# mika314/melonix

Measured on AMD Instinct MI355X. Metric: STFT+pitch+resynth frames/sec (48 kHz, 4096 FFT, 256 hop); % HBM roofline, higher is better.
Workload: dtype f32

## Files before the change

### melonix_amd/csrc/stft_core.h

```cpp
#pragma once
#include <stdint.h>
#include <type_traits>

#if defined(__HIPCC__)
#include <hip/hip_runtime.h>
#define MX_HD __host__ __device__ __forceinline__
namespace mx {
using cpx = float2;
}
#else
#define MX_HD inline __attribute__((always_inline))
namespace mx {
struct alignas(8) cpx {
  float x, y;
};
}
#endif

namespace mx {

#include "stft_consts.inc"

MX_HD cpx mk(float x, float y) {
  cpx r;
// ... 203 lines not shown
    for (int e = 0; e < P::E; ++e) {
      const cpx xs = ld_pair<ALIGNED8>(x, 2 * (t + P::T * e));
      Y[e] = pk_mul(xs, e < P::E - kGeoTail ? geo_weight<P, false>(a0, e) : geo_weight<P, true>(a0, e));
    }
  } else {
#pragma unroll
    for (int e = 0; e < P::E; ++e) Y[e] = pk_mul(ld_pair<ALIGNED8>(x, 2 * (t + P::T * e)), geo_weight<P, true>(a0, e));
  }
}

template <class P>
MX_HD void apply_window_geo(int t, cpx (&Y)[P::E], const cpx (&xr)[P::E], const float *wb, int hop) {
  const cpx a0 = ld_pair<true>(wb, 2 * t);
  if (geo_clamped_slots<P>(hop) <= kGeoTail) {
#pragma unroll
    for (int e = 0; e < P::E; ++e)
      Y[e] = pk_mul(xr[e], e < P::E - kGeoTail ? geo_weight<P, false>(a0, e) : geo_weight<P, true>(a0, e));
  } else {
#pragma unroll
    for (int e = 0; e < P::E; ++e) Y[e] = pk_mul(xr[e], geo_weight<P, true>(a0, e));
  }
}

template <class P, bool ALIGNED8>
MX_HD void load_raw(int t, cpx (&xr)[P::E], const float *x) {
#pragma unroll
  for (int e = 0; e < P::E; ++e) {
    xr[e] = ld_pair<ALIGNED8>(x, 2 * (t + P::T * e));
  }
}
template <class P, int WSTEP, bool ALIGNED8>
MX_HD void apply_window(int t, cpx (&Y)[P::E], const cpx (&xr)[P::E], const float *w) {
#pragma unroll
  for (int e = 0; e < P::E; ++e) {
    const int p = 2 * (t + P::T * e);
    cpx ws;
    if constexpr (WSTEP == 1) {
      ws = ld_pair<ALIGNED8>(w, p);
    } else {
      const f2u wu = *reinterpret_cast<const f2u *>(w - p - 1);
      ws = mk(wu.y, wu.x);
    }
    Y[e] = pk_mul(xr[e], ws);
  }
}

template <class P>
MX_HD void pass1(const cpx (&Y)[P::E], cpx (&v)[P::E]) {
#pragma unroll
  for (int b = 0; b < P::NB1; ++b) {
    cpx in[P::R1], out[P::R1];
#pragma unroll
    for (int r = 0; r < P::R1; ++r) in[r] = Y[b + P::NB1 * r];
    Dft<P::R1>::run(in, out);
#pragma unroll
    for (int r = 0; r < P::R1; ++r) v[b * P::R1 + r] = out[r];
  }
}

template <class P, int HOP>
struct Slide {
  static constexpr int H = HOP / 2;
  static constexpr bool ok = (HOP > 0) && (HOP % 2 == 0) && (H % P::T == 0) && (2 * (H / P::T) <= P::E);
  static constexpr int D = ok ? H / P::T : 1;
};

template <class P, int HOP>
MX_HD void slide_edge(int t, const float *wtab, float inv_sc, cpx (&edge)[Slide<P, HOP>::D]) {
  using S = Slide<P, HOP>;
#pragma unroll
  for (int i = 0; i < S::D; ++i) {
    const int p = 2 * (t + P::T * (P::E - 2 * S::D + i));
    edge[i] = mk(wtab[p] * inv_sc, wtab[p + 1] * inv_sc);
  }
}

template <class P, int HOP>
MX_HD void slide_fetch(int t, const float *xe, cpx (&nx)[Slide<P, HOP>::D]) {
  using S = Slide<P, HOP>;
#pragma unroll
  for (int i = 0; i < S::D; ++i) nx[i] = *reinterpret_cast<const cpx *>(xe - HOP + 2 * (t + P::T * i));
}

template <class P, int HOP>
MX_HD void slide_step(cpx (&Y)[P::E], const cpx (&nx)[Slide<P, HOP>::D], const cpx (&edge)[Slide<P, HOP>::D],
                      float g, float sc) {
  using S = Slide<P, HOP>;
  const cpx gg = mk(g, g), ss = mk(sc, sc);
#pragma unroll
  for (int e = 0; e < P::E - 2 * S::D; ++e) Y[e] = pk_mul_xs(Y[e + S::D], gg);
#pragma unroll
  for (int i = 0; i < S::D; ++i) Y[P::E - 2 * S::D + i] = pk_mul(Y[P::E - S::D + i], edge[i]);
#pragma unroll
  for (int i = 0; i < S::D; ++i) Y[P::E - S::D + i] = pk_mul_xs(nx[i], ss);
}


template <class P>
struct Circ {
  static constexpr int W = 2 * P::T;
  static constexpr int CS = (P::T == 128) ? 4 : (P::T == 256) ? 3 : 2;
  static MX_HD bool ok(int hop) { return hop >= 1 && hop <= (CS - 1) * P::T && hop <= 2 * W; }
  static constexpr int slot(int k) { return (P::E - (CS - 1) + k) & (P::E - 1); }
};
template <class P>
struct CircGeo {
  int o;
  int s;
  int cr;
  int len;
};
template <class P>
MX_HD CircGeo<P> circ_geo(long long frame_end, int hop) {
  constexpr int W = Circ<P>::W;
  const long long start = frame_end - P::N;
  CircGeo<P> g;
  g.o = (int)(start & (long long)(W - 1));
  g.s = ((int)((start - hop) & (long long)(W - 1)) + hop) / W;
  g.len = 2 * hop;
  g.cr = (g.o - g.len) & (P::N - 1);
  return g;
}
template <class P>
MX_HD void circ_load_first(int t, cpx (&Y)[P::E], const float *xa, const float *w, int o) {
#pragma unroll
  for (int e = 0; e < P::E; ++e) {
    const int c2 = 2 * (t + P::T * e);
    const int q0 = (c2 - o) & (P::N - 1), q1 = (c2 + 1 - o) & (P::N - 1);
    Y[e] = mk(xa[q0] * w[q0], xa[q1] * w[q1]);
  }
}
template <class P>
MX_HD void circ_fetch(int t, const float *xs, const float *wt, const CircGeo<P> &g, float (&px)[2 * Circ<P>::CS],
                      float (&pw)[2 * Circ<P>::CS]) {
#pragma unroll
  for (int k = 0; k < Circ<P>::CS; ++k) {
    const int c2 = 2 * (t + P::T * Circ<P>::slot(k));
    int d0 = (c2 - g.cr) & (P::N - 1), d1 = (c2 + 1 - g.cr) & (P::N - 1);
    d0 = d0 < g.len ? d0 : g.len - 1;
    d1 = d1 < g.len ? d1 : g.len - 1;
    px[2 * k] = ld_one(xs, d0);
    px[2 * k + 1] = ld_one(xs, d1);
    pw[2 * k] = ld_one(wt, d0);
    pw[2 * k + 1] = ld_one(wt, d1);
  }
}
template <class P, int S>
MX_HD void circ_age(cpx (&Y)[P::E], cpx gg) {
  cpx head[S > 0 ? S : 1];
#pragma unroll
  for (int i = 0; i < S; ++i) head[i] = Y[i];
#pragma unroll
  for (int e = 0; e < P::E - S; ++e) Y[e] = pk_mul_xs(Y[e + S], gg);
#pragma unroll
  for (int i = 0; i < S; ++i) Y[P::E - S + i] = pk_mul_xs(head[i], gg);
}
template <class P>
MX_HD void circ_step(int t, cpx (&Y)[P::E], float decay, const CircGeo<P> &g, const float (&px)[2 * Circ<P>::CS],
                     const float (&pw)[2 * Circ<P>::CS]) {
  const cpx gg = mk(decay, decay);
  constexpr int SMAX = (Circ<P>::W - 1 + (Circ<P>::CS - 1) * P::T) / Circ<P>::W;
  static_assert(SMAX <= 2, "rotations by 0, 1 or 2 slots");
  if (g.s == 0) circ_age<P, 0>(Y, gg);
  else if (SMAX == 1 || g.s == 1) circ_age<P, 1>(Y, gg);
  else circ_age<P, 2>(Y, gg);
#pragma unroll
  for (int k = 0; k < Circ<P>::CS; ++k) {
    const int e = Circ<P>::slot(k);
    const int c2 = 2 * (t + P::T * e);
    const int d0 = (c2 - g.cr) & (P::N - 1), d1 = (c2 + 1 - g.cr) & (P::N - 1);
    const float n0 = px[2 * k] * pw[2 * k], n1 = px[2 * k + 1] * pw[2 * k + 1];
    Y[e] = mk(d0 < g.len ? n0 : Y[e].x, d1 < g.len ? n1 : Y[e].y);
  }
}


#if defined(__HIP_DEVICE_COMPILE__)
#define MX_LDS_ASM 1
typedef float mx_f2v __attribute__((ext_vector_type(2)));
template <int OFF>
__device__ __forceinline__ mx_f2v lds_rd64(uint32_t addr) {
  static_assert(OFF >= 0 && OFF < 163840, "LDS is 160 KiB");
  mx_f2v r;
  if constexpr (OFF < 65536) {
    asm volatile("ds_read_b64 %0, %1 offset:%2" : "=v"(r) : "v"(addr), "n"(OFF) : "memory");
  } else {
    const uint32_t hi = addr + (uint32_t)(OFF & ~65535);
    asm volatile("ds_read_b64 %0, %1 offset:%2" : "=v"(r) : "v"(hi), "n"(OFF & 65535) : "memory");
  }
  return r;
}
__device__ __forceinline__ uint32_t lds_addr(const void *p) {
  return (uint32_t)(uintptr_t)(const __attribute__((address_space(3))) void *)p;
}
template <int N>
__device__ __forceinline__ void lds_wait(mx_f2v (&q)[N]) {
  static_assert(N % 8 == 0, "tied in groups of 8");
  asm volatile("s_waitcnt lgkmcnt(0)" ::: "memory");
#pragma unroll
  for (int i = 0; i < N; i += 8)
    asm volatile("" : "+v"(q[i]), "+v"(q[i + 1]), "+v"(q[i + 2]), "+v"(q[i + 3]), "+v"(q[i + 4]),
                 "+v"(q[i + 5]), "+v"(q[i + 6]), "+v"(q[i + 7]));
}
#endif
template <int I, int N, class F>
MX_HD void static_for(F &&f) {
  if constexpr (I < N) {
    f(std::integral_constant<int, I>{});
    static_for<I + 1, N>(f);
  }
}

template <class P>
MX_HD void store_t1(int t, const cpx (&v)[P::E], cpx *lds) {
  if constexpr (t1_padded<P>()) {
    static_assert(P::R1 <= 32 && (P::T * P::R1) % 32 == 0, "T1 padding is one point per 32");
    cpx *const p = lds + (t * P::R1 + ((t * P::R1) >> 5));
#pragma unroll
    for (int b = 0; b < P::NB1; ++b) {
#pragma unroll
      for (int r = 0; r < P::R1; ++r) p[b * (P::T * P::R1 + P::T * P::R1 / 32) + r] = v[b * P::R1 + r];
    }
  } else {
    const unsigned B8 = (unsigned)((t * P::R1) ^ (t & 15)) << 3;
    char *const base = reinterpret_cast<char *>(lds);
#pragma unroll
    for (int r = 0; r < P::R1; ++r) {
      cpx *p = reinterpret_cast<cpx *>(base + (B8 ^ ((unsigned)r << 3)));
#pragma unroll
      for (int b = 0; b < P::NB1; ++b) p[b * P::T * P::R1] = v[b * P::R1 + r];
    }
  }
}

template <class P>
struct T1Read {
  static constexpr int S = P::M / P::R2;
  static constexpr int SP = t1_padded<P>() ? S + S / 32 : S;
  static constexpr int TP = t1_padded<P>() ? P::T + P::T / 32 : P::T;
  static constexpr int step = t1_padded<P>() ? 0 : ((S >> P::L1) & 15);
  static_assert(S % 32 == 0 && P::T % 32 == 0 && (step == 0 || step == 8), "T1 read is base(+alt base) + offset");
  static_assert(t1_padded<P>() || P::NB2 == 1, "the XOR layout's bases are written for one pass-2 butterfly per thread");
};

template <class P>
MX_HD void load_t1(int t, cpx (&v)[P::E], const cpx *lds) {
  using R = T1Read<P>;
  const int s1 = t1_index<P>(t);
#ifdef MX_LDS_ASM
  mx_f2v q[P::E];
  const uint32_t ae = lds_addr(lds + s1), ao = lds_addr(lds + (s1 ^ R::step));
  static_for<0, P::NB2>([&](auto bb) {
    constexpr int b = decltype(bb)::value;
    static_for<0, P::R2>([&](auto rr) {
      constexpr int r = decltype(rr)::value;
      q[b * P::R2 + r] = lds_rd64<(b * R::TP + r * R::SP) * 8>((r & 1) ? ao : ae);
    });
  });
  lds_wait(q);
#pragma unroll
  for (int i = 0; i < P::E; ++i) v[i] = mk(q[i].x, q[i].y);
#else
  const cpx *pe = lds + s1, *po = lds + (s1 ^ R::step);
#pragma unroll
  for (int b = 0; b < P::NB2; ++b) {
#pragma unroll
    for (int r = 0; r < P::R2; ++r) v[b * P::R2 + r] = ((r & 1) ? po : pe)[b * R::TP + r * R::SP];
  }
#endif
}

template <class P>
MX_HD void load_t1_tw2(int t, cpx (&v)[P::E], const cpx *lds, const cpx *ltw2, cpx (&w)[P::R2 - 1]) {
  static_assert(P::NB2 == 1 && P::E == P::R2 && P::E % 8 == 0, "one pass-2 butterfly per thread");
  using R = T1Read<P>;
  const int s1 = t1_index<P>(t);
#ifdef MX_LDS_ASM
  const uint32_t ae = lds_addr(lds + s1), ao = lds_addr(lds + (s1 ^ R::step));
  const uint32_t aw = lds_addr(ltw2 + (t & (P::R1 - 1)));
  mx_f2v q[2 * P::E];
  static_for<0, P::R2>([&](auto rr) {
    constexpr int r = decltype(rr)::value;
    q[r] = lds_rd64<r * R::SP * 8>((r & 1) ? ao : ae);
  });
  static_for<1, P::R2>([&](auto rr) {
    constexpr int r = decltype(rr)::value;
    q[P::E + r] = lds_rd64<(r - 1) * P::R1 * 8>(aw);
  });
  q[P::E] = mx_f2v{0.0f, 0.0f};
  lds_wait(q);
#pragma unroll
  for (int i = 0; i < P::E; ++i) v[i] = mk(q[i].x, q[i].y);
#pragma unroll
  for (int r = 1; r < P::R2; ++r) w[r - 1] = mk(q[P::E + r].x, q[P::E + r].y);
#else
  const cpx *pe = lds + s1, *po = lds + (s1 ^ R::step), *pw = ltw2 + (t & (P::R1 - 1));
#pragma unroll
  for (int r = 0; r < P::R2; ++r) v[r] = ((r & 1) ? po : pe)[r * R::SP];
#pragma unroll
  for (int r = 1; r < P::R2; ++r) w[r - 1] = pw[(r - 1) * P::R1];
#endif
}

template <class P>
MX_HD void pass2(int t, cpx (&v)[P::E], const cpx *tw2) {
#pragma unroll
  for (int b = 0; b < P::NB2; ++b) {
    const int j = t + P::T * b;
    const int k = j & (P::R1 - 1);
    cpx in[P::R2], w[P::R2], out[P::R2];
    w[0] = mk(1.0f, 0.0f);
#pragma unroll
    for (int r = 0; r < P::R2; ++r) in[r] = v[b * P::R2 + r];
#pragma unroll
    for (int r = 1; r < P::R2; ++r) {
      w[r] = tw2[(r - 1) * P::R1 + k];
    }
    DftTw<P::R2, 1, 0, false>::run(in, w, out);
#pragma unroll
    for (int r = 0; r < P::R2; ++r) v[b * P::R2 + r] = out[r];
  }
}

template <class P>
MX_HD void pass2_reg(cpx (&v)[P::E], const cpx (&w)[P::R2 - 1]) {
  static_assert(P::NB2 == 1, "one pass-2 butterfly per thread");
  cpx in[P::R2], ww[P::R2], out[P::R2];
  ww[0] = mk(1.0f, 0.0f);
#pragma unroll
  for (int r = 0; r < P::R2; ++r) in[r] = v[r];
#pragma unroll
  for (int r = 1; r < P::R2; ++r) ww[r] = w[r - 1];
  DftTw<P::R2, 1, 0, false>::run(in, ww, out);
#pragma unroll
  for (int r = 0; r < P::R2; ++r) v[r] = out[r];
}

template <class P>
MX_HD void store_t2(int t, const cpx (&v)[P::E], cpx *lds) {
#pragma unroll
  for (int b = 0; b < P::NB2; ++b) {
    const int j = t + P::T * b;
    const int k = j & (P::R1 - 1);
    const int base = (j - k) * P::R2 + k;
    cpx *p = lds + base;
#pragma unroll
    for (int r = 0; r < P::R2; ++r) p[r * P::R1] = v[b * P::R2 + r];
  }
}

template <class P>
MX_HD int k0p(int t) { return t; }
template <class P>
MX_HD int k0q(int t) { return t ? P::NS3 - t : P::NS3 / 2; }

template <class P>
MX_HD void load_t2(int t, cpx (&v)[P::E], const cpx *lds) {
  const int p = k0p<P>(t), q = k0q<P>(t);
#ifdef MX_LDS_ASM
  {
    const uint32_t pa = lds_addr(lds + p), qa = lds_addr(lds + q);
    mx_f2v w[P::E];
    static_for<0, P::R3>([&](auto rr) {
      constexpr int r = decltype(rr)::value;
      w[r] = lds_rd64<P::NS3 * r * 8>(pa);
      w[P::R3 + r] = lds_rd64<P::NS3 * r * 8>(qa);
    });
    lds_wait(w);
#pragma unroll
    for (int i = 0; i < P::E; ++i) v[i] = mk(w[i].x, w[i].y);
  }
#else
  const cpx *pp = lds + p, *qq = lds + q;
#pragma unroll
  for (int r = 0; r < P::R3; ++r) {
    v[r] = pp[P::NS3 * r];
    v[P::R3 + r] = qq[P::NS3 * r];
  }
#endif
}

template <class P>
MX_HD constexpr int q_index(int r) { return P::R3 + ((r + 1) & (P::R3 - 1)); }

template <class P>
MX_HD void fetch_tw3(int t, const cpx *tw3, cpx (&w)[P::R3 - 1]) {
  const int col = t ? t : P::NS3 / 2;
#pragma unroll
  for (int r = 1; r < P::R3; ++r) w[r - 1] = tw3[(r - 1) * P::NS3 + col];
}
template <class P>
MX_HD void fetch_tw3_bases(int t, const cpx *tw3, cpx (&wb)[6]) {
  static_assert(P::R3 == 16, "two-level pass-3 twiddles are written for radix 16");
  const int col = t ? t : P::NS3 / 2;
  constexpr int rr[6] = {1, 2, 3, 4, 8, 12};
#pragma unroll
  for (int i = 0; i < 6; ++i) wb[i] = tw3[(rr[i] - 1) * P::NS3 + col];
}
template <class P, bool MAY0>
MX_HD void pass3_reg(int t, cpx (&v)[P::E], const cpx (&w)[P::R3 - 1]);
template <class P, bool MAY0 = true>
MX_HD void pass3_bases(int t, cpx (&v)[P::E], const cpx (&wb)[6]) {
  cpx w[P::R3 - 1];
#pragma unroll
  for (int r = 1; r < P::R3; ++r) {
    const int hi = r >> 2, lo = r & 3;
    if (hi == 0) w[r - 1] = wb[lo - 1];
    else if (lo == 0) w[r - 1] = wb[2 + hi];
    else w[r - 1] = pk_cmul2(wb[2 + hi], wb[lo - 1]);
  }
  pass3_reg<P, MAY0>(t, v, w);
}
template <class P, int KH>
MX_HD void pass3_wp0(int t, const cpx (&w)[P::R3 - 1], cpx (&wph)[KH > 0 ? KH : 1]) {
  static_assert(KH >= 0 && KH <= P::R3 - 1, "at most every twiddle");
  wph[0] = mk(1.0f, 0.0f);
#pragma unroll
  for (int r = 1; r <= KH; ++r) wph[r - 1] = csel(t == 0, mk(1.0f, 0.0f), w[r - 1]);
}
template <class P, bool MAY0 = true, int KH = 0>
MX_HD void pass3_reg(int t, cpx (&v)[P::E], const cpx (&w)[P::R3 - 1], const cpx (&wph)[KH > 0 ? KH : 1]) {
  constexpr int R = P::R3;
  const bool t0 = MAY0 && (t == 0);
  cpx inp[R], inq[R], wp[R], wq[R], out[R];
  wp[0] = wq[0] = mk(1.0f, 0.0f);
#pragma unroll
  for (int r = 0; r < R; ++r) {
    inp[r] = v[r];
    inq[r] = v[R + r];
  }
#pragma unroll
  for (int r = 1; r < R; ++r) {
    wp[r] = (MAY0 && r <= KH) ? wph[r <= KH ? r - 1 : 0] : csel(t0, mk(1.0f, 0.0f), w[r - 1]);
    wq[r] = w[r - 1];
  }
  DftTw<R, 1, 0, false>::run(inp, wp, out);
#pragma unroll
  for (int r = 0; r < R; ++r) v[r] = out[r];
  DftTw<R, 1, 0, true>::run(inq, wq, out);
#pragma unroll
  for (int r = 0; r < R; ++r) v[R + r] = out[r];
}
template <class P, bool MAY0>
MX_HD void pass3_reg(int t, cpx (&v)[P::E], const cpx (&w)[P::R3 - 1]) {
  const cpx none[1] = {mk(1.0f, 0.0f)};
  pass3_reg<P, MAY0, 0>(t, v, w, none);
}

template <class P, int S>
struct PostSlot {
  static MX_HD void run(bool t0, const cpx (&v)[P::E], const cpx (&u)[P::R3], float (&mg)[P::E]) {
    constexpr int R = P::R3, H = R / 2;
    cpx A, B;
    if constexpr (S < H) {
      A = csel(t0, v[q_index<P>(S)], v[S]);
      B = v[q_index<P>(R - 1 - S)];
    } else {
      A = csel(t0, v[S - H], v[S]);
      B = csel(t0, v[(3 * H - S) & (R - 1)], v[q_index<P>(R - 1 - S)]);
    }
    const cpx n2 = pk_split_norm2(A, B, u[S]);
    mg[2 * S] = fast_sqrt(n2.x);
    mg[2 * S + 1] = fast_sqrt(n2.y);
    if constexpr (S == H) {
      const cpx z = v[H];
      const float m = fast_sqrt(cnorm2(z)) * 2.0f;
      mg[2 * S + 1] = t0 ? m : mg[2 * S + 1];
    }
    if constexpr (S + 1 < R) PostSlot<P, S + 1>::run(t0, v, u, mg);
  }
};

template <class P, bool MAY0 = true>
MX_HD void post(int t, const cpx (&v)[P::E], const cpx (&u)[P::R3], float (&mg)[P::E]) {
  PostSlot<P, 0>::run(MAY0 && t == 0, v, u, mg);
}

template <class P, int S>
struct PostFly {
  static MX_HD void run(cpx lo, cpx hi, cpx (&u)[P::R3]) {
    constexpr int k = ((32 / P::R3) * S) % 64;
    const cpx b = S < P::R3 / 2 ? lo : hi;
    if constexpr (k == 0) u[S] = b;
    else if constexpr (k == 16) u[S] = mk(b.y, -b.x);
    else u[S] = pk_rot_cs(b, mk(kCos64[k], kSin64[k]));
    if constexpr (S + 1 < P::R3) PostFly<P, S + 1>::run(lo, hi, u);
  }
};
template <class P>
MX_HD void post_bases(int t, const cpx *ubase, cpx &lo, cpx &hi) {
  if (t) {
    lo = ubase[t];
    hi = lo;
  } else {
    constexpr int k = 16 / P::R3;
    lo = mk(kSin64[k], kCos64[k]);
    hi = mk(-1.0f, 0.0f);
  }
}
template <class P, bool MAY0 = true>
MX_HD void post_fly(int t, const cpx (&v)[P::E], cpx lo, cpx hi, float (&mg)[P::E]) {
  cpx u[P::R3];
  PostFly<P, 0>::run(lo, MAY0 ? hi : lo, u);
  PostSlot<P, 0>::run(MAY0 && t == 0, v, u, mg);
}

template <class P, int S>
struct PostSlotC {
  static MX_HD void run(bool t0, const cpx (&v)[P::E], const cpx (&u)[P::R3], cpx (&X)[P::E]) {
    constexpr int R = P::R3, H = R / 2;
    cpx A, B;
    if constexpr (S < H) {
      A = csel(t0, v[q_index<P>(S)], v[S]);
      B = v[q_index<P>(R - 1 - S)];
    } else {
      A = csel(t0, v[S - H], v[S]);
      B = csel(t0, v[(3 * H - S) & (R - 1)], v[q_index<P>(R - 1 - S)]);
    }
    const cpx Sm = pk_add_cj(A, B);
    const cpx Dm = pk_sub_cj(A, B);
    const cpx D = pk_cmul<false>(Dm, u[S]);
    X[2 * S] = pk_sub(Sm, D);
    X[2 * S + 1] = cconj(pk_add(Sm, D));
    if constexpr (S == H) {
      const cpx z = v[H];
      X[2 * S + 1] = csel(t0, mk(2.0f * z.x, -2.0f * z.y), X[2 * S + 1]);
    }
    if constexpr (S + 1 < R) PostSlotC<P, S + 1>::run(t0, v, u, X);
  }
};
template <class P, bool MAY0 = true>
MX_HD void post_cplx(int t, const cpx (&v)[P::E], const cpx (&u)[P::R3], cpx (&X)[P::E]) {
  PostSlotC<P, 0>::run(MAY0 && t == 0, v, u, X);
}

template <class P>
MX_HD void out_bases(int t, int &lo, int &hi) {
  lo = t ? t : P::NS3 / 2;
  hi = t ? t : -(P::R3 / 2) * P::NS3;
}
template <class P>
MX_HD int out_bin(int t, int o) {
  int lo, hi;
  out_bases<P>(t, lo, hi);
  const int s = o >> 1;
  int k = (s < P::R3 / 2 ? lo : hi) + P::NS3 * s;
  if (o & 1) {
    k = P::M - k;
    if (k == P::M) k = P::M / 2;
  }
  return k;
}
template <class P>
MX_HD uint32_t band_mask(int t, int kmin, int kmax) {
  uint32_t m = 0;
#pragma unroll
  for (int o = 0; o < P::E; ++o) {
    const int k = out_bin<P>(t, o);
    m |= (k >= kmin && k <= kmax) ? (1u << o) : 0u;
  }
  return m;
}
MX_HD unsigned long long pick_key(float mag, int bin, bool in_band) {
  const unsigned in = in_band ? 0xffffffffu : 0u;
  return ((unsigned long long)(__builtin_bit_cast(unsigned, mag) & in) << 32) | ((0x7fffffffu - (unsigned)bin) & in);
}
MX_HD unsigned long long pick_key(float mag, int bin, int kmin, int kmax) {
  return pick_key(mag, bin, bin >= kmin && bin <= kmax);
}
MX_HD unsigned long long row_pick_key(int b0, float m0, float m1, float m2, float m3, int kmin, int kmax) {
  unsigned long long best = pick_key(m0, b0, kmin, kmax);
  const unsigned long long k1 = pick_key(m1, b0 + 1, kmin, kmax), k2 = pick_key(m2, b0 + 2, kmin, kmax),
                           k3 = pick_key(m3, b0 + 3, kmin, kmax);
  best = k1 > best ? k1 : best;
  best = k2 > best ? k2 : best;
  best = k3 > best ? k3 : best;
  return best;
}
MX_HD unsigned long long row_pick_key(int b0, float m0, float m1, float m2, float m3, bool in0, bool in1, bool in2, bool in3) {
  unsigned long long best = pick_key(m0, b0, in0);
  const unsigned long long k1 = pick_key(m1, b0 + 1, in1), k2 = pick_key(m2, b0 + 2, in2), k3 = pick_key(m3, b0 + 3, in3);
  best = k1 > best ? k1 : best;
  best = k2 > best ? k2 : best;
  best = k3 > best ? k3 : best;
  return best;
}
MX_HD unsigned row_band_mask(int b0, int kmin, int kmax) {
  unsigned m = 0;
#pragma unroll
  for (int j = 0; j < 4; ++j) m |= (b0 + j >= kmin && b0 + j <= kmax) ? (1u << j) : 0u;
  return m;
}
MX_HD unsigned long long row_pick_key(int b0, float m0, float m1, float m2, float m3, unsigned mask) {
  return row_pick_key(b0, m0, m1, m2, m3, (mask & 1u) != 0, (mask & 2u) != 0, (mask & 4u) != 0, (mask & 8u) != 0);
}

template <class P, int S>
struct PostTw {
  static MX_HD void run(cpx lo, cpx hi, cpx (&u)[P::R3]) {
    u[S] = mulw64<(32 / P::R3) * S>(S < P::R3 / 2 ? lo : hi);
    if constexpr (S + 1 < P::R3) PostTw<P, S + 1>::run(lo, hi, u);
  }
};
template <class P>
MX_HD void post_twiddles(int t, const cpx *ubase, cpx (&u)[P::R3]) {
  cpx lo, hi;
  if (t) {
    lo = ubase[t];
    hi = lo;
  } else {
    constexpr int k = 16 / P::R3;
    lo = mk(kSin64[k], kCos64[k]);
    hi = mk(-1.0f, 0.0f);
  }
  PostTw<P, 0>::run(lo, hi, u);
}

}
```

### melonix_amd/csrc/stft_kernel_impl.h

```cpp
#pragma once
#include <hip/hip_runtime.h>

#include "colormap_core.h"
#include "kernels.h"
#include "stft_core.h"
#include "stft_tables.h"

#define MX_BARRIER() __syncthreads()

namespace mx {

template <bool MAXOP>
__device__ __forceinline__ unsigned wave_reduce_u32(unsigned k) {
  constexpr unsigned ident = MAXOP ? 0u : 0xffffffffu;
#define MX_DPP_STEP(CTRL, ROWS)                                                                      \
  {                                                                                                  \
    const unsigned o = (unsigned)__builtin_amdgcn_update_dpp((int)ident, (int)k, CTRL, ROWS, 0xf, false); \
    k = MAXOP ? (o > k ? o : k) : (o < k ? o : k);                                                   \
  }
  MX_DPP_STEP(0xB1, 0xf)
  MX_DPP_STEP(0x4E, 0xf)
  MX_DPP_STEP(0x141, 0xf)
  MX_DPP_STEP(0x140, 0xf)
  MX_DPP_STEP(0x142, 0xa)
  MX_DPP_STEP(0x143, 0xc)
#undef MX_DPP_STEP
  return (unsigned)__builtin_amdgcn_readlane((int)k, 63);
}
__device__ __forceinline__ unsigned long long wave_max_u64(unsigned long long k) {
  const unsigned hi = (unsigned)(k >> 32), lo = (unsigned)k;
  const unsigned mhi = wave_reduce_u32<true>(hi);
  const unsigned long long tie = __ballot(hi == mhi);
  unsigned mlo;
  if (__builtin_popcountll(tie) == 1) mlo = (unsigned)__builtin_amdgcn_readlane((int)lo, __builtin_ctzll(tie));
  else mlo = wave_reduce_u32<true>(hi == mhi ? lo : 0u);
  return ((unsigned long long)mhi << 32) | mlo;
}

template <int IMM, bool NT = true>
__device__ __forceinline__ void st_row_nt(const float *base, unsigned off, float x) {
  static_assert(IMM >= -4096 && IMM <= 4095, "global_store immediate offset");
#if defined(__HIP_DEVICE_COMPILE__)
  if constexpr (NT) asm volatile("global_store_dword %0, %1, %2 offset:%3 nt" : : "v"(off), "v"(x), "s"(base), "n"(IMM) : "memory");
  else asm volatile("global_store_dword %0, %1, %2 offset:%3" : : "v"(off), "v"(x), "s"(base), "n"(IMM) : "memory");
#endif
}

template <class P, int MODE, int HOP, int WPE, bool DEFER = false, bool PREFETCH = false, bool CMAP = false, bool DIRECT = false,
          bool CIRC = false, bool ROWPICK = false>
__global__ __launch_bounds__(P::T) __attribute__((amdgpu_waves_per_eu(WPE, WPE)))
void stft_kernel(const StftArgs a0) {
  const StftArgs &a = a0;
  using C = P;
  constexpr int N = P::N;
  constexpr int NW = C::T / 64;
  constexpr int kRed = (NW > 1) ? ((NW + 1) / 2) * 2 : 0;
  constexpr bool kTw3Bases = (P::R3 == 16);
  constexpr int kTw2 = ((C::TW2 + 1) / 2) * 2;
  static_assert(P::R3 == 16 || P::R3 == 8, "twiddle placement per plan");
  static_assert(!DIRECT || (NW > 1 && !DEFER && !CMAP), "direct row stores: multi-wave, non-deferred plans");
  static_assert(!ROWPICK || (DEFER && NW > 1 && !CMAP && !DIRECT && C::M / 4 / C::T >= 1 && C::T >= 128),
                "row-side pitch pick: the deferred two-wave plan, rows without texels");
  static_assert(!CIRC || (MODE != kRanges && HOP == 0 && !PREFETCH && !CMAP), "circular window: bulk modes");
  constexpr int IMG = t1_size<C>();
  __shared__ __attribute__((aligned(16))) float2 lds[IMG + kRed + (DEFER ? C::M / 2 : 0) + kTw2];
  float *const lout = reinterpret_cast<float *>(DEFER ? lds + IMG : lds);
  float2 *const ltw2 = lds + IMG + kRed + (DEFER ? C::M / 2 : 0);

  const int t_ = threadIdx.x;
  constexpr bool kSlide = (MODE == kBulkAligned) && (HOP > 0) && Slide<P, (HOP > 0 ? HOP : 2)>::ok;
  constexpr int SD = Slide<P, (HOP > 0 ? HOP : 2)>::D;
  const bool wave0 = __builtin_amdgcn_readfirstlane(t_) < 64;
  cpx u[kTw3Bases ? 1 : P::R3];
  cpx ulo;
  cpx w3r[kTw3Bases ? 1 : P::R3 - 1], w3base[6];
  if constexpr (kTw3Bases) {
    cpx uhi_unused;
    post_bases<P>(t_, a.ubase, ulo, uhi_unused);
    fetch_tw3_bases<P>(t_, a.tw3, w3base);
  } else {
    post_twiddles<P>(t_, a.ubase, *reinterpret_cast<cpx(*)[P::R3]>(&u));
    fetch_tw3<P>(t_, a.tw3, *reinterpret_cast<cpx(*)[P::R3 - 1]>(&w3r));
  }
  constexpr int kTw3Hoist = (!kTw3Bases && ROWPICK) ? ((kSlide && SD > 1) ? 3 : P::R3 - 1) : 0;
  cpx w3p[kTw3Hoist > 0 ? kTw3Hoist : 1];
  if constexpr (!kTw3Bases) pass3_wp0<P, kTw3Hoist>(t_, *reinterpret_cast<cpx(*)[P::R3 - 1]>(&w3r), w3p);
  uint32_t bmask_ = 0;
  uint32_t umask = 0;
  if constexpr (!ROWPICK) {
    bmask_ = band_mask<P>(t_, a.kmin, a.kmax);
#pragma unroll
    for (int o = 0; o < P::E; ++o) umask |= (__ballot((bmask_ >> o) & 1u) != 0ull) ? (1u << o) : 0u;
    umask = __builtin_amdgcn_readfirstlane(umask);
  }
  unsigned long long rin[4] = {0ull, 0ull, 0ull, 0ull};
  if constexpr (ROWPICK) {
    const unsigned rm = row_band_mask(4 * t_, a.kmin, a.kmax);
#pragma unroll
    for (int j = 0; j < 4; ++j) rin[j] = __ballot((rm >> j) & 1u);
  }
  constexpr float kSc = 0.5f / (float)N;
  for (int i = t_; i < C::TW2; i += C::T) ltw2[i] = a.tw2[i];
  MX_BARRIER();

  unsigned lb = blockIdx.x;
  {
    const unsigned nb = gridDim.x, xcd = lb & 7u, q = nb >> 3, r = nb & 7u;
    lb = (xcd < r ? xcd * (q + 1) : r * (q + 1) + (xcd - r) * q) + (lb >> 3);
  }
  const int64_t f0 = (int64_t)lb * a.frames_per_block;
  const int64_t f1 = (f0 + a.frames_per_block < a.count) ? f0 + a.frames_per_block : a.count;

  cpx Y[P::E];
  cpx edge[SD], nx[SD];
  if constexpr (kSlide) {
    const int64_t e0 = (a.first_frame + f0 + 1) * (int64_t)HOP;
    if (f0 < f1) load_frame<P, 1, true>(t_, Y, a.audio + MX_AUDIO_PAD + (e0 - N), a.wtab);
    slide_edge<P, HOP>(t_, a.wtab, 2.0f * (float)N, edge);
  }

  unsigned long long *const red = reinterpret_cast<unsigned long long *>(lds + IMG + (DEFER ? C::M / 2 : 0));
  auto flush_pitch = [&](int64_t fr, int tt) {
    if (!ROWPICK && a.pitch && tt == 0) {
      unsigned long long b = red[0];
#pragma unroll
      for (int i = 1; i < NW; ++i) b = red[i] > b ? red[i] : b;
      mx_pitch p;
      p.bin = 0x7fffffff - (int)(unsigned)(b & 0xffffffffull);
      p.mag = __uint_as_float((unsigned)(b >> 32));
      a.pitch[fr] = p;
    }
  };
  const bool want_rows = a.mags != nullptr || (CMAP && a.rgb != nullptr);
  constexpr bool kRowSaddr = (C::M / 4 / C::T == 4) && (C::T * 16 == 2048);
  auto flush_row = [&](int64_t fr, int tt) {
    if (want_rows) {
      using f32x4 = float __attribute__((ext_vector_type(4)));
      const f32x4 *l4 = reinterpret_cast<const f32x4 *>(lout) + tt;
      f32x4 *row4 = reinterpret_cast<f32x4 *>(a.mags + (size_t)fr * (size_t)(N / 2)) + tt;
      f32x4 q[C::M / 4 / C::T];
#pragma unroll
      for (int i = 0; i < C::M / 4 / C::T; ++i) q[i] = l4[C::T * i];
      if (!CMAP || a.mags) {
        if constexpr (kRowSaddr) {
          uintptr_t mid = reinterpret_cast<uintptr_t>(a.mags + (size_t)fr * (size_t)(N / 2)) + 4096;
#if defined(__HIP_DEVICE_COMPILE__)
          asm volatile("" : "+s"(mid));
          using gchar = __attribute__((address_space(1))) char;
          using gf32x4 = __attribute__((address_space(1))) f32x4;
#else
          using gchar = char;
          using gf32x4 = f32x4;
#endif
          const unsigned off = 16u * (unsigned)tt;
#pragma unroll
          for (int i = 0; i < 4; ++i)
            __builtin_nontemporal_store(q[i], reinterpret_cast<gf32x4 *>(reinterpret_cast<gchar *>(mid) + off + (2048 * i - 4096)));
        } else {
#pragma unroll
          for (int i = 0; i < C::M / 4 / C::T; ++i) {
            __builtin_nontemporal_store(q[i], &row4[C::T * i]);
          }
        }
      }
      if constexpr (ROWPICK) {
        if (wave0) {
          const unsigned long long b = wave_max_u64(row_pick_key(
              4 * tt, q[0].x, q[0].y, q[0].z, q[0].w, __builtin_amdgcn_inverse_ballot_w64(rin[0]),
              __builtin_amdgcn_inverse_ballot_w64(rin[1]), __builtin_amdgcn_inverse_ballot_w64(rin[2]),
              __builtin_amdgcn_inverse_ballot_w64(rin[3])));
          if (tt == 0) {
            mx_pitch p;
            p.bin = 0x7fffffff - (int)(unsigned)(b & 0xffffffffull);
            p.mag = __uint_as_float((unsigned)(b >> 32));
            a.pitch[fr] = p;
          }
        }
      }
      if constexpr (CMAP) {
        if (a.rgb) {
          uint32_t *trow = reinterpret_cast<uint32_t *>(a.rgb + (size_t)fr * (size_t)(N / 2) * 3) + 3 * tt;
#pragma unroll 1
          for (int i = 0; i < C::M / 4 / C::T; ++i) {
            uint32_t w3[3];
            texel4(q[i].x, q[i].y, q[i].z, q[i].w, a.cmap_k, w3);
            uint32_t *o = trow + 3 * C::T * i;
            o[0] = w3[0];
            o[1] = w3[1];
            o[2] = w3[2];
          }
        }
      }
    }
  };

  auto frame_ptrs = [&](int64_t fr, int zo, const float *&x, const float *&w) {
    if constexpr (MODE == kRanges) {
      const int s = a.ranges[2 * fr], e = a.ranges[2 * fr + 1];
      const bool outside = (e <= 0) || ((int64_t)e - N >= a.n);
      x = outside ? a.audio : a.audio + MX_AUDIO_PAD + ((int64_t)e - N);
      int64_t d0 = (int64_t)N - ((int64_t)e - (int64_t)s);
      d0 = d0 < (int64_t)(N - 1 - kWOff) ? (int64_t)(N - 1 - kWOff) : d0;
      d0 = d0 > (int64_t)(kWDmax + kWTail) ? (int64_t)(kWDmax + kWTail) : d0;
      w = a.wext + kWOff + d0;
    } else {
      const int64_t e = (a.first_frame + fr + 1) * (int64_t)a.hop;
      x = a.audio + MX_AUDIO_PAD + (e - N);
      w = a.wtab + zo;
    }
  };
  float cpx_[2 * Circ<P>::CS], cpw_[2 * Circ<P>::CS];
  if constexpr (CIRC) {
    if (f0 < f1) {
      const int64_t pe = (a.first_frame + f0 + 1) * (int64_t)a.hop;
      circ_load_first<P>(t_, Y, a.audio + MX_AUDIO_PAD + (pe - N), a.wtab, circ_geo<P>(pe, a.hop).o);
    }
  }
  cpx xr[(PREFETCH && !kSlide) ? P::E : 1];
  if constexpr (PREFETCH && !kSlide) {
    if (f0 < f1) {
      const float *x0;
      const float *w0;
      frame_ptrs(f0, 0, x0, w0);
      load_raw<P, (MODE == kBulkAligned)>(t_, xr, x0);
    }
  }

  for (int64_t f = f0; f < f1; ++f) {
    int t = t_;
    unsigned bmask = bmask_;
    int zoff = 0;
    asm volatile("" : "+v"(t), "+v"(bmask), "+s"(zoff));
    int out_lo, out_hi;
    out_bases<P>(t, out_lo, out_hi);

    if constexpr (CIRC) {
      if (f > f0) {
        const int64_t pe = (a.first_frame + f + 1) * (int64_t)a.hop;
        const CircGeo<P> geo = circ_geo<P>(pe, a.hop);
        circ_fetch<P>(t, a.audio + MX_AUDIO_PAD + (pe - 2 * (int64_t)a.hop), a.wtab + zoff + (N - 2 * a.hop), geo, cpx_, cpw_);
        circ_step<P>(t, Y, a.decay, geo, cpx_, cpw_);
      }
    } else if constexpr (kSlide) {
      if (f > f0) slide_step<P, HOP>(Y, nx, edge, a.decay, kSc);
      if (f + 1 < f1) slide_fetch<P, HOP>(t, a.audio + MX_AUDIO_PAD + (a.first_frame + f + 2) * (int64_t)HOP, nx);
    } else {
      const float *x;
      const float *w;
      frame_ptrs(f, zoff, x, w);
      if constexpr (PREFETCH) {
        if constexpr (MODE == kRanges) apply_window<P, -1, false>(t, Y, xr, w);
        else apply_window_geo<P>(t, Y, xr, a.wtab + N + zoff, a.hop);
      } else if constexpr (MODE == kRanges) {
        load_frame<P, -1, false>(t, Y, x, w);
      } else {
        load_frame_geo<P, (MODE == kBulkAligned)>(t, Y, x, a.wtab + N + zoff, a.hop);
      }
    }

    cpx v[P::E];
    pass1<P>(Y, v);
    constexpr bool kTw2Batch = (P::NB2 == 1);
    store_t1<P>(t, v, lds);
    MX_BARRIER();
    if constexpr (DEFER || DIRECT) {
      if (f > f0) flush_pitch(f - 1, t);
    }
    if constexpr (kTw2Batch) {
      cpx w2[P::R2 - 1];
      load_t1_tw2<P>(t, v, lds, ltw2, w2);
      if constexpr (DEFER) {
        if (f > f0) flush_row(f - 1, t);
      }
      MX_BARRIER();
      pass2_reg<P>(v, w2);
    } else {
      load_t1<P>(t, v, lds);
      if constexpr (DEFER) {
        if (f > f0) flush_row(f - 1, t);
      }
      MX_BARRIER();
      pass2<P>(t, v, ltw2);
    }
    store_t2<P>(t, v, lds);
    MX_BARRIER();
    load_t2<P>(t, v, lds);
    MX_BARRIER();
    float mg[P::E];
    if (NW == 1 || wave0) {
      if constexpr (kTw3Bases) {
        pass3_bases<P, true>(t, v, w3base);
        post_fly<P, true>(t, v, ulo, csel(t == 0, mk(-1.0f, 0.0f), ulo), mg);
      } else {
        pass3_reg<P, true, kTw3Hoist>(t, v, *reinterpret_cast<cpx(*)[P::R3 - 1]>(&w3r), w3p);
        post<P, true>(t, v, *reinterpret_cast<cpx(*)[P::R3]>(&u), mg);
      }
    } else {
      if constexpr (kTw3Bases) {
        pass3_bases<P, false>(t, v, w3base);
        post_fly<P, false>(t, v, ulo, ulo, mg);
      } else {
        pass3_reg<P, false>(t, v, *reinterpret_cast<cpx(*)[P::R3 - 1]>(&w3r));
        post<P, false>(t, v, *reinterpret_cast<cpx(*)[P::R3]>(&u), mg);
      }
    }

    if constexpr (PREFETCH && !kSlide) {
      if (f + 1 < f1) {
        const float *xn;
        const float *wn;
        frame_ptrs(f + 1, zoff, xn, wn);
        load_raw<P, (MODE == kBulkAligned)>(t, xr, xn);
      }
    }

    unsigned long long best = 0ull;
    if (!ROWPICK && a.pitch) {
      const unsigned klo = 0x7fffffffu - (unsigned)out_lo, khi = 0x7fffffffu - (unsigned)out_hi;
      const unsigned nlo = 0x7fffffffu - (unsigned)(C::M - out_lo), nhi = 0x7fffffffu - (unsigned)(C::M - out_hi);
#pragma unroll
      for (int s = 0; s < C::R3; ++s) {
        constexpr int H = C::R3 / 2;
        if (!((umask >> (2 * s)) & 3u)) continue;
        const unsigned b0 = (s < H ? klo : khi) - (unsigned)(C::NS3 * s);
        unsigned b1 = (s < H ? nlo : nhi) + (unsigned)(C::NS3 * s);
        if (s == H) b1 = (t == 0) ? 0x7fffffffu - (unsigned)(C::M / 2) : b1;
        const unsigned v0 = (unsigned)((int)(bmask << (31 - 2 * s)) >> 31);
        const unsigned v1 = (unsigned)((int)(bmask << (31 - (2 * s + 1))) >> 31);
        const unsigned long long k0 = ((unsigned long long)(__float_as_uint(mg[2 * s]) & v0) << 32) | (b0 & v0);
        const unsigned long long k1 = ((unsigned long long)(__float_as_uint(mg[2 * s + 1]) & v1) << 32) | (b1 & v1);
        best = k0 > best ? k0 : best;
        best = k1 > best ? k1 : best;
      }
      best = wave_max_u64(best);
      if constexpr (NW > 1) {
        if ((t & 63) == 0) red[t >> 6] = best;
      }
    }

    if constexpr (DIRECT) {
      if (want_rows) {
        const float *row = a.mags + (size_t)f * (size_t)(N / 2);
        constexpr int H = C::R3 / 2;
        constexpr int STEP = 4 * C::NS3;
        constexpr int G = 8192 / STEP;
        static_assert((STEP == 4096 || STEP == 2048) && H % G == 0, "slot groups share an offset through the store's immediate");
        const unsigned blo = 4u * (unsigned)out_lo, bhi = 4u * (unsigned)(out_hi + C::NS3 * H);
        const unsigned nlo = 4u * (unsigned)(C::M - out_lo), nhi = 4u * (unsigned)(C::M - out_hi - C::NS3 * H);
        static_for<0, C::R3>([&](auto ss) {
          constexpr int s = decltype(ss)::value;
          constexpr int sl = s < H ? s : s - H;
          constexpr int su = (sl & ~(G - 1)) + G / 2, sd = (sl & ~(G - 1)) + G / 2 - 1;
          const unsigned o0 = (s < H ? blo : bhi) + (unsigned)(su * STEP);
          unsigned o1 = (s < H ? nlo : nhi) - (unsigned)(sd * STEP);
          if constexpr (s == H) {
            o1 = (t == 0) ? (unsigned)(4 * (C::M / 2)) + (unsigned)((sl - sd) * STEP) : o1;
          }
          st_row_nt<(sl - su) * STEP>(row, o0, mg[2 * s]);
          st_row_nt<-(sl - sd) * STEP, false>(row, o1, mg[2 * s + 1]);
        });
      }
    } else if (want_rows) {
      float *plo = lout + out_lo, *phi = lout + out_hi;
      float *mlo = lout + (C::M - out_lo), *mhi = lout + (C::M - out_hi);
      constexpr int H = C::R3 / 2;
#pragma unroll
      for (int s = 0; s < C::R3; ++s) (s < H ? plo : phi)[C::NS3 * s] = mg[2 * s];
#pragma unroll
      for (int s = 0; s < C::R3; ++s)
        if (s != H) (s < H ? mlo : mhi)[-C::NS3 * s] = mg[2 * s + 1];
      (t == 0 ? lout + C::M / 2 : mhi - C::NS3 * H)[0] = mg[2 * H + 1];
    }
    if constexpr (!DEFER && !DIRECT) {
      if (want_rows) {
        MX_BARRIER();
        flush_row(f, t);
        MX_BARRIER();
      } else {
        MX_BARRIER();
      }
      if constexpr (NW > 1) {
        flush_pitch(f, t);
      } else if (a.pitch && t == 0) {
        mx_pitch p;
        p.bin = 0x7fffffff - (int)(unsigned)(best & 0xffffffffull);
        p.mag = __uint_as_float((unsigned)(best >> 32));
        a.pitch[f] = p;
      }
    }
  }
  if constexpr (DEFER || DIRECT) {
    if (f0 < f1) {
      MX_BARRIER();
      flush_pitch(f1 - 1, t_);
      if constexpr (DEFER) flush_row(f1 - 1, t_);
    }
  }
}


}
```

### melonix_amd/csrc/stft_kernels.hip

```cpp
#include <hip/hip_runtime.h>

#include "kernels.h"
#include "stft_kernel_impl.h"

namespace mx {

namespace {

template <class P>
struct Tune {
  static constexpr bool TWO_WAVE = (P::E == 16);
  static constexpr int WPE = TWO_WAVE ? 3 : 2;
  static constexpr bool PREFETCH = (P::E == 32);
  static constexpr bool slides(int hop) {
    return P::N == 4096 ? (hop == 256 || hop == 512) : P::N == 16384 ? (hop == 512 || hop == 1024) : hop == 1024;
  }
  static constexpr bool DIRECT = (P::N >= 16384);
  static constexpr bool CIRC = (P::N >= 16384);
  static constexpr bool DEFER = TWO_WAVE;
};

template <class P, int HOP, bool ROWPICK = false>
bool try_slide(const StftArgs &b, dim3 grid, dim3 block, hipStream_t s) {
  if constexpr (Slide<P, HOP>::ok && Tune<P>::slides(HOP)) {
    if (b.hop != HOP) return false;
    hipLaunchKernelGGL((stft_kernel<P, kBulkAligned, HOP, Tune<P>::WPE, Tune<P>::DEFER, false, false, Tune<P>::DIRECT, false, ROWPICK>),
                       grid, block, 0, s, b);
    return true;
  } else {
    return false;
  }
}

template <class P>
bool try_circ(const StftArgs &b, dim3 grid, dim3 block, hipStream_t s) {
  if constexpr (!Tune<P>::CIRC) {
    return false;
  } else {
    if (!Circ<P>::ok(b.hop)) return false;
    hipLaunchKernelGGL((stft_kernel<P, kBulkAny, 0, Tune<P>::WPE, Tune<P>::DEFER, false, false, Tune<P>::DIRECT, true>),
                       grid, block, 0, s, b);
    return true;
  }
}

template <class P>
hipError_t launch_plan(int mode, const StftArgs &a, hipStream_t s) {
  if (a.count <= 0) return hipSuccess;
  const int g = a.frames_per_block > 0 ? a.frames_per_block : 1;
  const int64_t blocks = (a.count + g - 1) / g;
  if (blocks > 0x7fffffffLL) return hipErrorInvalidValue;
  StftArgs b = a;
  b.frames_per_block = g;
  const dim3 grid((unsigned)blocks), block(P::T);
  constexpr int W = Tune<P>::WPE;
  constexpr bool DF = Tune<P>::DEFER, PF = Tune<P>::PREFETCH, DR = Tune<P>::DIRECT;
  if constexpr (DF) {
    if (mode != kRanges && !a.rgb && a.mags && a.pitch && 0 <= a.kmin && a.kmin <= a.kmax && a.kmax < 4 * 64) {
      if (mode == kBulkAny)
        hipLaunchKernelGGL((stft_kernel<P, kBulkAny, 0, W, DF, PF, false, DR, false, true>), grid, block, 0, s, b);
      else if (mode != kBulkAligned)
        return hipErrorInvalidValue;
      else if (!(try_slide<P, 256, true>(b, grid, block, s) || try_slide<P, 512, true>(b, grid, block, s)))
        hipLaunchKernelGGL((stft_kernel<P, kBulkAligned, 0, W, DF, PF, false, DR, false, true>), grid, block, 0, s, b);
      return hipGetLastError();
    }
  }
  switch (mode) {
    case kBulkAligned:
      if (!(try_slide<P, 256>(b, grid, block, s) || try_slide<P, 512>(b, grid, block, s) ||
            try_slide<P, 1024>(b, grid, block, s) || try_circ<P>(b, grid, block, s)))
        hipLaunchKernelGGL((stft_kernel<P, kBulkAligned, 0, W, DF, PF, false, DR>), grid, block, 0, s, b);
      break;
    case kBulkAny:
      if (try_circ<P>(b, grid, block, s)) break;
      hipLaunchKernelGGL((stft_kernel<P, kBulkAny, 0, W, DF, PF, false, DR>), grid, block, 0, s, b); break;
    case kRanges:
      if (a.rgb) hipLaunchKernelGGL((stft_kernel<P, kRanges, 0, (W > 2 ? 2 : W), DF, false, true>), grid, block, 0, s, b);
      else hipLaunchKernelGGL((stft_kernel<P, kRanges, 0, W, DF, false, false, DR>), grid, block, 0, s, b);
      break;
    default: return hipErrorInvalidValue;
  }
  return hipGetLastError();
}

}

int stft_points_per_thread(int N) { return N == 4096 ? kPlan4096E : 32; }

int stft_frames_per_block_cap(int N, int mode, int hop) {
  if (N == 32768 && mode != kRanges && Tune<Plan<32768, 32>>::CIRC && !Tune<Plan<32768, 32>>::slides(hop) &&
      Circ<Plan<32768, 32>>::ok(hop))
    return 32;
  return N == 32768 ? 8 : (N == 4096 ? 32 : 16);
}

hipError_t launch_stft(int N, int mode, const StftArgs &a, hipStream_t s) {
  switch (N) {
    case 4096: return launch_plan<Plan<4096, kPlan4096E>>(mode, a, s);
    case 16384: return launch_plan<Plan<16384, 32>>(mode, a, s);
    case 32768: return launch_plan<Plan<32768, 32>>(mode, a, s);
  }
  return hipErrorInvalidValue;
}

}
```

Baseline: 341.1 million.

## Use q-major padded LDS image for pass-2 and register-resident tail twiddles

Adds a q-major transpose image (pitch 130) for the N=4096 row-pick kernels, so pass-2 reads are strided by 8 rows with padding to avoid LDS bank conflicts. Only 13 twiddle rows are staged in LDS; the remaining pass-2 twiddles are fetched once into registers, shrinking LDS traffic. The pitch pick now reduces a 32-bit lane max and recovers the bin via ballot/readlane instead of a 64-bit key reduction. Risks include added register pressure and slightly different tie-breaking semantics.

```diff
diff --git a/melonix_amd/csrc/stft_core.h b/melonix_amd/csrc/stft_core.h
--- a/melonix_amd/csrc/stft_core.h
+++ b/melonix_amd/csrc/stft_core.h
@@ -529,6 +529,72 @@
 #endif
 }
 
+constexpr int kT1qPitch = 130;
+constexpr int kT1qTwRows = 13;
+template <class P>
+MX_HD constexpr int t1q_size() { return P::R1 * kT1qPitch; }
+MX_HD constexpr int t1q_index(int j, int q) { return q * kT1qPitch + j; }
+template <class P>
+MX_HD void store_t1q(int t, const cpx (&v)[P::E], cpx *lds) {
+  static_assert(P::NB1 == 1 && P::R1 == 16 && P::T <= kT1qPitch, "the q-major image is written for the N = 4096 plan");
+  cpx *const p = lds + t;
+#ifdef MX_LDS_ASM
+  volatile __attribute__((address_space(3))) mx_f2v *const lp = (volatile __attribute__((address_space(3))) mx_f2v *)p;
+#pragma unroll
+  for (int q = 0; q < P::R1; ++q) lp[q * kT1qPitch] = mx_f2v{v[q].x, v[q].y};
+#else
+#pragma unroll
+  for (int q = 0; q < P::R1; ++q) p[q * kT1qPitch] = v[q];
+#endif
+}
+template <class P>
+MX_HD void fetch_tw2_tail(int t, const cpx *tw2, cpx (&wt)[P::R2 - 1 - kT1qTwRows]) {
+#pragma unroll
+  for (int r = kT1qTwRows + 1; r < P::R2; ++r) wt[r - 1 - kT1qTwRows] = tw2[(r - 1) * P::R1 + (t & (P::R1 - 1))];
+}
+#ifdef MX_LDS_ASM
+__device__ __forceinline__ void lds_wait29(mx_f2v (&q)[29]) {
+  asm volatile("s_waitcnt lgkmcnt(0)" ::: "memory");
+#pragma unroll
+  for (int i = 0; i < 24; i += 8)
+    asm volatile("" : "+v"(q[i]), "+v"(q[i + 1]), "+v"(q[i + 2]), "+v"(q[i + 3]), "+v"(q[i + 4]),
+                 "+v"(q[i + 5]), "+v"(q[i + 6]), "+v"(q[i + 7]));
+  asm volatile("" : "+v"(q[24]), "+v"(q[25]), "+v"(q[26]), "+v"(q[27]), "+v"(q[28]));
+}
+#endif
+template <class P>
+MX_HD void load_t1q_tw2(int t, cpx (&v)[P::E], const cpx *lds, const cpx *ltw2, const cpx (&wt)[P::R2 - 1 - kT1qTwRows],
+                        cpx (&w)[P::R2 - 1]) {
+  static_assert(P::NB2 == 1 && P::E == P::R2 && P::R2 == 16 && P::M / P::R2 == 8 * P::R1, "one pass-2 butterfly per thread, j = a + 8 r");
+  const int b1 = kT1qPitch * (t & (P::R1 - 1)) + (t >> P::L1);
+#ifdef MX_LDS_ASM
+  const uint32_t ab = lds_addr(lds + b1);
+  const uint32_t aw = lds_addr(ltw2 + (t & (P::R1 - 1)));
+  mx_f2v q[P::E + kT1qTwRows];
+  static_for<0, P::R2>([&](auto rr) {
+    constexpr int r = decltype(rr)::value;
+    q[r] = lds_rd64<r * 8 * 8>(ab);
+  });
+  static_for<1, kT1qTwRows + 1>([&](auto rr) {
+    constexpr int r = decltype(rr)::value;
+    q[P::E + r - 1] = lds_rd64<(r - 1) * P::R1 * 8>(aw);
+  });
+  lds_wait29(q);
+#pragma unroll
+  for (int i = 0; i < P::E; ++i) v[i] = mk(q[i].x, q[i].y);
+#pragma unroll
+  for (int r = 1; r <= kT1qTwRows; ++r) w[r - 1] = mk(q[P::E + r - 1].x, q[P::E + r - 1].y);
+#else
+  const cpx *pb = lds + b1, *pw = ltw2 + (t & (P::R1 - 1));
+#pragma unroll
+  for (int r = 0; r < P::R2; ++r) v[r] = pb[8 * r];
+#pragma unroll
+  for (int r = 1; r <= kT1qTwRows; ++r) w[r - 1] = pw[(r - 1) * P::R1];
+#endif
+#pragma unroll
+  for (int r = kT1qTwRows + 1; r < P::R2; ++r) w[r - 1] = wt[r - 1 - kT1qTwRows];
+}
+
 template <class P>
 MX_HD void pass2(int t, cpx (&v)[P::E], const cpx *tw2) {
 #pragma unroll
@@ -822,6 +888,16 @@
   return row_pick_key(b0, m0, m1, m2, m3, (mask & 1u) != 0, (mask & 2u) != 0, (mask & 4u) != 0, (mask & 8u) != 0);
 }
 
+MX_HD unsigned row_pick_lane_max(float m0, float m1, float m2, float m3, bool in0, bool in1, bool in2, bool in3) {
+  const unsigned a = in0 ? __builtin_bit_cast(unsigned, m0) : 0u, b = in1 ? __builtin_bit_cast(unsigned, m1) : 0u;
+  const unsigned c = in2 ? __builtin_bit_cast(unsigned, m2) : 0u, d = in3 ? __builtin_bit_cast(unsigned, m3) : 0u;
+  const unsigned ab = a > b ? a : b, abc = ab > c ? ab : c;
+  return abc > d ? abc : d;
+}
+MX_HD int row_pick_first(unsigned mhi, unsigned b0, unsigned b1, unsigned b2, unsigned b3, bool in0, bool in1, bool in2, bool in3) {
+  return (in0 && b0 == mhi) ? 0 : (in1 && b1 == mhi) ? 1 : (in2 && b2 == mhi) ? 2 : 3;
+}
+
 template <class P, int S>
 struct PostTw {
   static MX_HD void run(cpx lo, cpx hi, cpx (&u)[P::R3]) {
diff --git a/melonix_amd/csrc/stft_kernel_impl.h b/melonix_amd/csrc/stft_kernel_impl.h
--- a/melonix_amd/csrc/stft_kernel_impl.h
+++ b/melonix_amd/csrc/stft_kernel_impl.h
@@ -47,7 +47,7 @@
 }
 
 template <class P, int MODE, int HOP, int WPE, bool DEFER = false, bool PREFETCH = false, bool CMAP = false, bool DIRECT = false,
-          bool CIRC = false, bool ROWPICK = false>
+          bool CIRC = false, bool ROWPICK = false, bool T1Q = false>
 __global__ __launch_bounds__(P::T) __attribute__((amdgpu_waves_per_eu(WPE, WPE)))
 void stft_kernel(const StftArgs a0) {
   const StftArgs &a = a0;
@@ -56,13 +56,16 @@
   constexpr int NW = C::T / 64;
   constexpr int kRed = (NW > 1) ? ((NW + 1) / 2) * 2 : 0;
   constexpr bool kTw3Bases = (P::R3 == 16);
-  constexpr int kTw2 = ((C::TW2 + 1) / 2) * 2;
+  constexpr int kTw2N = T1Q ? kT1qTwRows * P::R1 : C::TW2;
+  constexpr int kTw2 = ((kTw2N + 1) / 2) * 2;
   static_assert(P::R3 == 16 || P::R3 == 8, "twiddle placement per plan");
   static_assert(!DIRECT || (NW > 1 && !DEFER && !CMAP), "direct row stores: multi-wave, non-deferred plans");
   static_assert(!ROWPICK || (DEFER && NW > 1 && !CMAP && !DIRECT && C::M / 4 / C::T >= 1 && C::T >= 128),
                 "row-side pitch pick: the deferred two-wave plan, rows without texels");
+  static_assert(!T1Q || (ROWPICK && P::NB2 == 1 && P::R1 == 16), "q-major T1 image: the N = 4096 row-side-pick kernels");
   static_assert(!CIRC || (MODE != kRanges && HOP == 0 && !PREFETCH && !CMAP), "circular window: bulk modes");
-  constexpr int IMG = t1_size<C>();
+  constexpr int IMG = T1Q ? t1q_size<C>() : t1_size<C>();
+  static_assert(!DEFER || (IMG * 8) % 256 == 0, "the row region starts on a multiple of 256 bytes");
   __shared__ __attribute__((aligned(16))) float2 lds[IMG + kRed + (DEFER ? C::M / 2 : 0) + kTw2];
   float *const lout = reinterpret_cast<float *>(DEFER ? lds + IMG : lds);
   float2 *const ltw2 = lds + IMG + kRed + (DEFER ? C::M / 2 : 0);
@@ -99,8 +102,11 @@
 #pragma unroll
     for (int j = 0; j < 4; ++j) rin[j] = __ballot((rm >> j) & 1u);
   }
+  [[maybe_unused]] const unsigned long long rany = rin[0] | rin[1] | rin[2] | rin[3];
   constexpr float kSc = 0.5f / (float)N;
-  for (int i = t_; i < C::TW2; i += C::T) ltw2[i] = a.tw2[i];
+  for (int i = t_; i < kTw2N; i += C::T) ltw2[i] = a.tw2[i];
+  cpx w2t[T1Q ? P::R2 - 1 - kT1qTwRows : 1];
+  if constexpr (T1Q) fetch_tw2_tail<P>(t_, a.tw2, *reinterpret_cast<cpx(*)[P::R2 - 1 - kT1qTwRows]>(&w2t));
   MX_BARRIER();
 
   unsigned lb = blockIdx.x;
@@ -165,14 +171,22 @@
       }
       if constexpr (ROWPICK) {
         if (wave0) {
-          const unsigned long long b = wave_max_u64(row_pick_key(
-              4 * tt, q[0].x, q[0].y, q[0].z, q[0].w, __builtin_amdgcn_inverse_ballot_w64(rin[0]),
-              __builtin_amdgcn_inverse_ballot_w64(rin[1]), __builtin_amdgcn_inverse_ballot_w64(rin[2]),
-              __builtin_amdgcn_inverse_ballot_w64(rin[3])));
+          const unsigned m = row_pick_lane_max(q[0].x, q[0].y, q[0].z, q[0].w, __builtin_amdgcn_inverse_ballot_w64(rin[0]),
+                                               __builtin_amdgcn_inverse_ballot_w64(rin[1]), __builtin_amdgcn_inverse_ballot_w64(rin[2]),
+                                               __builtin_amdgcn_inverse_ballot_w64(rin[3]));
+          const unsigned mhi = wave_reduce_u32<true>(m);
+          const unsigned long long cand = __ballot(m == mhi) & rany;
+          const int L = __builtin_ctzll(cand);
+          const unsigned b0 = (unsigned)__builtin_amdgcn_readlane((int)__float_as_uint(q[0].x), L);
+          const unsigned b1 = (unsigned)__builtin_amdgcn_readlane((int)__float_as_uint(q[0].y), L);
+          const unsigned b2 = (unsigned)__builtin_amdgcn_readlane((int)__float_as_uint(q[0].z), L);
+          const unsigned b3 = (unsigned)__builtin_amdgcn_readlane((int)__float_as_uint(q[0].w), L);
+          const int j = row_pick_first(mhi, b0, b1, b2, b3, (rin[0] >> L) & 1ull, (rin[1] >> L) & 1ull, (rin[2] >> L) & 1ull,
+                                       (rin[3] >> L) & 1ull);
           if (tt == 0) {
             mx_pitch p;
-            p.bin = 0x7fffffff - (int)(unsigned)(b & 0xffffffffull);
-            p.mag = __uint_as_float((unsigned)(b >> 32));
+            p.bin = 4 * L + j;
+            p.mag = __uint_as_float(mhi);
             a.pitch[fr] = p;
           }
         }
@@ -261,14 +275,16 @@
     cpx v[P::E];
     pass1<P>(Y, v);
     constexpr bool kTw2Batch = (P::NB2 == 1);
-    store_t1<P>(t, v, lds);
+    if constexpr (T1Q) store_t1q<P>(t, v, lds);
+    else store_t1<P>(t, v, lds);
     MX_BARRIER();
     if constexpr (DEFER || DIRECT) {
       if (f > f0) flush_pitch(f - 1, t);
     }
     if constexpr (kTw2Batch) {
       cpx w2[P::R2 - 1];
-      load_t1_tw2<P>(t, v, lds, ltw2, w2);
+      if constexpr (T1Q) load_t1q_tw2<P>(t, v, lds, ltw2, *reinterpret_cast<cpx(*)[P::R2 - 1 - kT1qTwRows]>(&w2t), w2);
+      else load_t1_tw2<P>(t, v, lds, ltw2, w2);
       if constexpr (DEFER) {
         if (f > f0) flush_row(f - 1, t);
       }
diff --git a/melonix_amd/csrc/stft_kernels.hip b/melonix_amd/csrc/stft_kernels.hip
--- a/melonix_amd/csrc/stft_kernels.hip
+++ b/melonix_amd/csrc/stft_kernels.hip
@@ -20,11 +20,11 @@
   static constexpr bool DEFER = TWO_WAVE;
 };
 
-template <class P, int HOP, bool ROWPICK = false>
+template <class P, int HOP, bool ROWPICK = false, bool T1Q = false>
 bool try_slide(const StftArgs &b, dim3 grid, dim3 block, hipStream_t s) {
   if constexpr (Slide<P, HOP>::ok && Tune<P>::slides(HOP)) {
     if (b.hop != HOP) return false;
-    hipLaunchKernelGGL((stft_kernel<P, kBulkAligned, HOP, Tune<P>::WPE, Tune<P>::DEFER, false, false, Tune<P>::DIRECT, false, ROWPICK>),
+    hipLaunchKernelGGL((stft_kernel<P, kBulkAligned, HOP, Tune<P>::WPE, Tune<P>::DEFER, false, false, Tune<P>::DIRECT, false, ROWPICK, T1Q>),
                        grid, block, 0, s, b);
     return true;
   } else {
@@ -58,11 +58,11 @@
   if constexpr (DF) {
     if (mode != kRanges && !a.rgb && a.mags && a.pitch && 0 <= a.kmin && a.kmin <= a.kmax && a.kmax < 4 * 64) {
       if (mode == kBulkAny)
-        hipLaunchKernelGGL((stft_kernel<P, kBulkAny, 0, W, DF, PF, false, DR, false, true>), grid, block, 0, s, b);
+        hipLaunchKernelGGL((stft_kernel<P, kBulkAny, 0, W, DF, PF, false, DR, false, true, true>), grid, block, 0, s, b);
       else if (mode != kBulkAligned)
         return hipErrorInvalidValue;
-      else if (!(try_slide<P, 256, true>(b, grid, block, s) || try_slide<P, 512, true>(b, grid, block, s)))
-        hipLaunchKernelGGL((stft_kernel<P, kBulkAligned, 0, W, DF, PF, false, DR, false, true>), grid, block, 0, s, b);
+      else if (!(try_slide<P, 256, true, true>(b, grid, block, s) || try_slide<P, 512, true, true>(b, grid, block, s)))
+        hipLaunchKernelGGL((stft_kernel<P, kBulkAligned, 0, W, DF, PF, false, DR, false, true, true>), grid, block, 0, s, b);
       return hipGetLastError();
     }
   }
```

Measured after the change: 348.3 million, median of 6. +2.1%, better.
